# GLAD-RUC/DistEGNN

Hardware: NVIDIA H100
Metric: graph_steps_per_sec (higher is better)
Workload: dtype f32

## Files before the change

distegnn_b200/csrc/tc16.cuh:

```cuda
#pragma once
#include <cuda_fp16.h>

#include <type_traits>

#include "common.cuh"
#include "tile_mma.cuh"

namespace degnn {
namespace tc16 {

constexpr float RANGE = 3.0e4f;
__device__ __forceinline__ void split_pair(f32x2 x, uint32_t& hi, uint32_t& lo) {
    float x0, x1, l0, l1;
    upk2(x, x0, x1);
    const __half2 h = __floats2half2_rn(x0, x1);
    hi = *reinterpret_cast<const uint32_t*>(&h);
    const float2 hf = __half22float2(h);
    upk2(sub2(x, pk2(hf.x, hf.y)), l0, l1);
    const __half2 l = __floats2half2_rn(l0, l1);
    lo = *reinterpret_cast<const uint32_t*>(&l);
}

template <int NTHREADS, bool TRANSPOSED = false>
__device__ __forceinline__ void stage_weight(__half* hi, __half* lo, const float* __restrict__ wt_kmajor, int n_off,
                                             int n_total, int tid, float scale = 1.0f) {
    static_assert((H * H) % NTHREADS == 0, "thread count must divide the matrix");
    constexpr int R = H * H / NTHREADS;
    const uint32_t lbo_h = (uint32_t)(n_total / 8) * 64u;
    float w[R];
#pragma unroll
    for (int r = 0; r < R; ++r) w[r] = __ldg(wt_kmajor + tid + r * NTHREADS);
#pragma unroll
    for (int r = 0; r < R; ++r) {
        const int i = tid + r * NTHREADS;
        const int k = TRANSPOSED ? i & 63 : i >> 6, n = (TRANSPOSED ? i >> 6 : i & 63) + n_off;
        const float ws = w[r] * scale;
        const __half h = __float2half_rn(ws);
        const uint32_t o = (uint32_t)(k >> 3) * lbo_h + (uint32_t)(n >> 3) * 64u + (uint32_t)(n & 7) * 8u + (k & 7);
        hi[o] = h;
        lo[o] = __float2half_rn(ws - __half2float(h));
    }
}
__host__ __device__ constexpr uint32_t lbo_bytes(int n_total) { return (uint32_t)(n_total / 8) * 128u; }

template <uint32_t LBO, bool ACCUMULATE = false>
__device__ __forceinline__ void mma_f16x3_rA(float (&d)[32], const uint32_t (&a_hi)[16], const uint32_t (&a_lo)[16],
                                             uint64_t b_hi, uint64_t b_lo) {
    constexpr uint64_t B_KSTEP = (2 * LBO) >> 4;
    auto mma = [&](auto acc, const uint32_t (&a)[16], int ks, uint64_t b) {
        tmma::wgmma_f16_m64n64k16_rA<decltype(acc)::value>(d, a[4 * ks], a[4 * ks + 1], a[4 * ks + 2], a[4 * ks + 3],
                                                            b + ks * B_KSTEP);
    };
    tmma::wgmma_fence();
    mma(std::integral_constant<bool, ACCUMULATE>{}, a_lo, 0, b_hi);
#pragma unroll
    for (int ks = 1; ks < 4; ++ks) mma(std::true_type{}, a_lo, ks, b_hi);
#pragma unroll
    for (int ks = 0; ks < 4; ++ks) mma(std::true_type{}, a_hi, ks, b_lo);
#pragma unroll
    for (int ks = 0; ks < 4; ++ks) mma(std::true_type{}, a_hi, ks, b_hi);
    tmma::wgmma_commit();
}
__device__ __forceinline__ void mma_f16x3_rA_wait(float (&d)[32], uint32_t (&a_hi)[16], uint32_t (&a_lo)[16]) {
    tmma::wgmma_wait_all();
#pragma unroll
    for (int i = 0; i < 32; ++i) tmma::wgmma_keep(d[i]);
#pragma unroll
    for (int i = 0; i < 16; ++i) {
        tmma::wgmma_keep(a_hi[i]);
        tmma::wgmma_keep(a_lo[i]);
    }
}

__device__ __forceinline__ bool row_overflow(__half2 mx) {
    return fmaxf(__low2float(mx), __high2float(mx)) > RANGE;
}
__device__ __forceinline__ float range_scale(float rowmax) {
    const uint32_t eb = (__float_as_uint(rowmax) >> 23) & 0xffu;
    const uint32_t sb = eb > 141u ? 268u - eb : 127u;
    return __uint_as_float((sb < 1u ? 1u : sb) << 23);
}
__device__ __forceinline__ float quad_max(float v) {
    v = fmaxf(v, __shfl_xor_sync(FULL, v, 1));
    return fmaxf(v, __shfl_xor_sync(FULL, v, 2));
}
__device__ __forceinline__ float quad_sum(float v) {
    v += __shfl_xor_sync(FULL, v, 1);
    return v + __shfl_xor_sync(FULL, v, 2);
}

struct RowScales {
    float a = 1.0f, b = 1.0f, inv_a = 1.0f, inv_b = 1.0f;
};
constexpr int FAST_PASS = 0, MAX_PASS = 1, ENCODE_PASS = 2;
template <int P>
using Pass = std::integral_constant<int, P>;
struct NoGuard {
    __device__ __forceinline__ bool operator()() const { return false; }
};

template <bool SCALES_IN, bool ROLLED_MAX = false, class F, class Guard = NoGuard>
__device__ __forceinline__ void encode_rows(F&& f, uint32_t (&hi)[16], uint32_t (&lo)[16], RowScales& s,
                                            Guard&& guard = Guard{}) {
    bool cold = SCALES_IN && __any_sync(FULL, s.a != 1.0f || s.b != 1.0f);
    if (!cold) {
        __half2 mx = __floats2half2_rn(0.f, 0.f);
#pragma unroll
        for (int j = 0; j < 8; ++j) {
            f32x2 xa, xb;
            f(j, xa, xb, Pass<FAST_PASS>{});
            split_pair(xa, hi[2 * j], lo[2 * j]);
            split_pair(xb, hi[2 * j + 1], lo[2 * j + 1]);
            mx = __hmax2(mx, __habs2(*reinterpret_cast<const __half2*>(&hi[2 * j])));
            mx = __hmax2(mx, __habs2(*reinterpret_cast<const __half2*>(&hi[2 * j + 1])));
        }
        cold = __any_sync(FULL, row_overflow(mx) || guard());
    }
    if (!cold) return;
    float fa = 0.f, fb = 0.f;
    auto row_max = [&](int j) {
        f32x2 xa, xb;
        float v0, v1;
        f(j, xa, xb, Pass<MAX_PASS>{});
        upk2(xa, v0, v1);
        fa = fmaxf(fa, fmaxf(fabsf(v0), fabsf(v1)));
        upk2(xb, v0, v1);
        fb = fmaxf(fb, fmaxf(fabsf(v0), fabsf(v1)));
    };
    if constexpr (ROLLED_MAX) {
#pragma unroll 1
        for (int j = 0; j < 8; ++j) row_max(j);
    } else {
#pragma unroll
        for (int j = 0; j < 8; ++j) row_max(j);
    }
    float ca = range_scale(quad_max(fa)), ia = 1.0f / ca;
    float cb = range_scale(quad_max(fb)), ib = 1.0f / cb;
    if constexpr (SCALES_IN) {
        ca = fminf(ca, s.a);
        cb = fminf(cb, s.b);
        ia = 1.0f / ca;
        ib = 1.0f / cb;
    }
    s = {ca, cb, ia, ib};
#pragma unroll
    for (int j = 0; j < 8; ++j) {
        f32x2 xa, xb;
        f(j, xa, xb, Pass<ENCODE_PASS>{});
        split_pair(mul2(xa, bc2(s.a)), hi[2 * j], lo[2 * j]);
        split_pair(mul2(xb, bc2(s.b)), hi[2 * j + 1], lo[2 * j + 1]);
    }
}

__device__ __forceinline__ void phi_head_t(const float (&d)[32], float inv_a, float inv_b, const float* b, const float* w,
                                           int q, float& phia, float& phib) {
    float qmax = 0.f;
    f32x2 pha, phb;
    auto pass = [&](auto safe) {
        pha = phb = bc2(0.f);
#pragma unroll
        for (int j = 0; j < 8; ++j) {
            const f32x2 bb = *reinterpret_cast<const f32x2*>(b + 8 * j + 2 * q);
            const f32x2 ww = *reinterpret_cast<const f32x2*>(w + 8 * j + 2 * q);
            f32x2 sa = fma2(pk2(d[4 * j + 0], d[4 * j + 1]), bc2(inv_a), bb);
            f32x2 sb = fma2(pk2(d[4 * j + 2], d[4 * j + 3]), bc2(inv_b), bb);
            silu4t<decltype(safe)::value>(sa, sb, qmax);
            pha = fma2(sa, ww, pha);
            phb = fma2(sb, ww, phb);
        }
    };
    pass(std::false_type{});
    if (__any_sync(FULL, silu_q_overflow(qmax))) pass(std::true_type{});
    float p0, p1;
    upk2(pha, p0, p1);
    phia = quad_sum(p0 + p1);
    upk2(phb, p0, p1);
    phib = quad_sum(p0 + p1);
}

}
}
```

distegnn_b200/csrc/tile_mma.cuh:

```cuda
#pragma once
#include <cuda_runtime.h>
#include <stdint.h>

namespace degnn {

extern __shared__ __align__(1024) uint8_t degnn_dyn_smem[];

namespace tmma {

constexpr uint32_t TM_COLGROUP_BYTES = 2048;
__host__ __device__ constexpr int tm_bytes(int ncols) { return ncols * 128 * 4; }

__device__ __forceinline__ uint32_t smem_u32(const void* p) {
    return (uint32_t)__cvta_generic_to_shared(p);
}

__device__ __forceinline__ uint32_t tm_addr_rc(uint32_t row, uint32_t col) {
    return smem_u32(degnn_dyn_smem) + (col >> 2) * TM_COLGROUP_BYTES + row * 16u + (col & 3u) * 4u;
}
__device__ __forceinline__ uint32_t tm_addr(uint32_t taddr) {
    return tm_addr_rc((taddr >> 16) + (threadIdx.x & 31u), taddr & 0xffffu);
}

__device__ __forceinline__ uint64_t make_desc(uint32_t smem_addr, uint32_t lbo, uint32_t sbo) {
    return (uint64_t)((smem_addr >> 4) & 0x3FFF) | ((uint64_t)((lbo >> 4) & 0x3FFF) << 16) |
           ((uint64_t)((sbo >> 4) & 0x3FFF) << 32);
}

__device__ __forceinline__ void fence_proxy_async_smem() { asm volatile("fence.proxy.async.shared::cta;" ::: "memory"); }

__device__ __forceinline__ void tm_st4(uint32_t taddr, const uint32_t (&r)[4]) {
    asm volatile("st.shared.v4.b32 [%0], {%1,%2,%3,%4};" ::"r"(tm_addr(taddr)), "r"(r[0]), "r"(r[1]), "r"(r[2]), "r"(r[3])
                 : "memory");
}
__device__ __forceinline__ void tm_ld4(uint32_t taddr, uint32_t* r) {
    asm volatile("ld.shared.v4.b32 {%0,%1,%2,%3}, [%4];" : "=r"(r[0]), "=r"(r[1]), "=r"(r[2]), "=r"(r[3]) : "r"(tm_addr(taddr))
                 : "memory");
}
__device__ __forceinline__ void tm_st8(uint32_t taddr, const uint32_t (&r)[8]) {
    tm_st4(taddr, *reinterpret_cast<const uint32_t(*)[4]>(&r[0]));
    tm_st4(taddr + 4, *reinterpret_cast<const uint32_t(*)[4]>(&r[4]));
}
__device__ __forceinline__ void tm_st16(uint32_t taddr, const uint32_t (&r)[16]) {
#pragma unroll
    for (int i = 0; i < 4; ++i) tm_st4(taddr + 4 * i, *reinterpret_cast<const uint32_t(*)[4]>(&r[4 * i]));
}
__device__ __forceinline__ void tm_ld16(uint32_t taddr, uint32_t (&r)[16]) {
#pragma unroll
    for (int i = 0; i < 4; ++i) tm_ld4(taddr + 4 * i, &r[4 * i]);
}
__device__ __forceinline__ void prefetch_l1(const void* p) { asm volatile("prefetch.global.L1 [%0];" ::"l"(p)); }
__device__ __forceinline__ void prefetch_l2(const void* p) { asm volatile("prefetch.global.L2 [%0];" ::"l"(p)); }

__device__ __forceinline__ void wgmma_fence() { asm volatile("wgmma.fence.sync.aligned;" ::: "memory"); }
__device__ __forceinline__ void wgmma_commit() { asm volatile("wgmma.commit_group.sync.aligned;" ::: "memory"); }
__device__ __forceinline__ void wgmma_wait_all() { asm volatile("wgmma.wait_group.sync.aligned 0;" ::: "memory"); }
__device__ __forceinline__ void wgmma_f16_m64n64k16(float (&d)[32], uint64_t a_desc, uint64_t b_desc, uint32_t accumulate) {
    asm volatile(
        "{\n\t"
        ".reg .pred p;\n\t"
        "setp.ne.b32 p, %34, 0;\n\t"
        "wgmma.mma_async.sync.aligned.m64n64k16.f32.f16.f16 "
        "{%0,%1,%2,%3,%4,%5,%6,%7,%8,%9,%10,%11,%12,%13,%14,%15,%16,%17,%18,%19,%20,%21,%22,%23,%24,%25,%26,%27,%28,%29,%30,%31},"
        " %32, %33, p, 1, 1, 0, 0;\n\t"
        "}\n"
        : "+f"(d[0]), "+f"(d[1]), "+f"(d[2]), "+f"(d[3]), "+f"(d[4]), "+f"(d[5]), "+f"(d[6]), "+f"(d[7]), "+f"(d[8]),
          "+f"(d[9]), "+f"(d[10]), "+f"(d[11]), "+f"(d[12]), "+f"(d[13]), "+f"(d[14]), "+f"(d[15]), "+f"(d[16]),
          "+f"(d[17]), "+f"(d[18]), "+f"(d[19]), "+f"(d[20]), "+f"(d[21]), "+f"(d[22]), "+f"(d[23]), "+f"(d[24]),
          "+f"(d[25]), "+f"(d[26]), "+f"(d[27]), "+f"(d[28]), "+f"(d[29]), "+f"(d[30]), "+f"(d[31])
        : "l"(a_desc), "l"(b_desc), "r"(accumulate)
        : "memory");
}
#define DEGNN_WGMMA_RA_D(c)                                                                                             \
    c(d[0]), c(d[1]), c(d[2]), c(d[3]), c(d[4]), c(d[5]), c(d[6]), c(d[7]), c(d[8]), c(d[9]), c(d[10]), c(d[11]),      \
        c(d[12]), c(d[13]), c(d[14]), c(d[15]), c(d[16]), c(d[17]), c(d[18]), c(d[19]), c(d[20]), c(d[21]), c(d[22]),  \
        c(d[23]), c(d[24]), c(d[25]), c(d[26]), c(d[27]), c(d[28]), c(d[29]), c(d[30]), c(d[31])
#define DEGNN_WGMMA_RA_ASM(scale_d)                                                                                     \
    "wgmma.mma_async.sync.aligned.m64n64k16.f32.f16.f16 "                                                               \
    "{%0,%1,%2,%3,%4,%5,%6,%7,%8,%9,%10,%11,%12,%13,%14,%15,%16,%17,%18,%19,%20,%21,%22,%23,%24,%25,%26,%27,%28,%29,%30," \
    "%31}, {%32,%33,%34,%35}, %36, " scale_d ", 1, 1, 0;\n"
template <bool ACCUMULATE>
__device__ __forceinline__ void wgmma_f16_m64n64k16_rA(float (&d)[32], uint32_t a0, uint32_t a1, uint32_t a2, uint32_t a3,
                                                       uint64_t b_desc) {
    if (ACCUMULATE)
        asm volatile(DEGNN_WGMMA_RA_ASM("1") : DEGNN_WGMMA_RA_D("+f")
                     : "r"(a0), "r"(a1), "r"(a2), "r"(a3), "l"(b_desc) : "memory");
    else
        asm volatile(DEGNN_WGMMA_RA_ASM("0") : DEGNN_WGMMA_RA_D("=f")
                     : "r"(a0), "r"(a1), "r"(a2), "r"(a3), "l"(b_desc) : "memory");
}
#undef DEGNN_WGMMA_RA_D
#undef DEGNN_WGMMA_RA_ASM
__device__ __forceinline__ void wgmma_keep(float& r) { asm volatile("" : "+f"(r)::"memory"); }
__device__ __forceinline__ void wgmma_keep(uint32_t& r) { asm volatile("" : "+r"(r)::"memory"); }
__device__ __forceinline__ void frag_rows(int mb, uint32_t& r0, uint32_t& q) {
    const uint32_t w = (threadIdx.x >> 5) & 3u, l = threadIdx.x & 31u;
    r0 = 64u * (uint32_t)mb + 16u * w + (l >> 2);
    q = l & 3u;
}
__device__ __forceinline__ void frag_store(const float (&d)[32], uint32_t col, int mb) {
    uint32_t r0, q;
    frag_rows(mb, r0, q);
#pragma unroll
    for (int j = 0; j < 8; ++j) {
        const uint32_t c = col + 8u * j + 2u * q;
        const uint32_t a0 = tm_addr_rc(r0, c), a1 = tm_addr_rc(r0 + 8u, c);
        asm volatile("st.shared.v2.f32 [%0], {%1,%2};" ::"r"(a0), "f"(d[4 * j]), "f"(d[4 * j + 1]) : "memory");
        asm volatile("st.shared.v2.f32 [%0], {%1,%2};" ::"r"(a1), "f"(d[4 * j + 2]), "f"(d[4 * j + 3]) : "memory");
    }
}
__device__ __forceinline__ void frag_load(float (&d)[32], uint32_t col, int mb) {
    uint32_t r0, q;
    frag_rows(mb, r0, q);
#pragma unroll
    for (int j = 0; j < 8; ++j) {
        const uint32_t c = col + 8u * j + 2u * q;
        asm volatile("ld.shared.v2.f32 {%0,%1}, [%2];" : "=f"(d[4 * j]), "=f"(d[4 * j + 1]) : "r"(tm_addr_rc(r0, c)) : "memory");
        asm volatile("ld.shared.v2.f32 {%0,%1}, [%2];" : "=f"(d[4 * j + 2]), "=f"(d[4 * j + 3]) : "r"(tm_addr_rc(r0 + 8u, c))
                     : "memory");
    }
}

__device__ __forceinline__ void mbar_init(uint64_t* bar, uint32_t count) {
    asm volatile("mbarrier.init.shared::cta.b64 [%0], %1;" ::"r"(smem_u32(bar)), "r"(count) : "memory");
}
__device__ __forceinline__ void fence_mbar_init() { asm volatile("fence.mbarrier_init.release.cluster;" ::: "memory"); }
__device__ __forceinline__ void mbar_expect_tx(uint64_t* bar, uint32_t bytes) {
    asm volatile("mbarrier.arrive.expect_tx.shared::cta.b64 _, [%0], %1;" ::"r"(smem_u32(bar)), "r"(bytes) : "memory");
}
__device__ __forceinline__ void mbar_wait(uint64_t* bar, uint32_t parity) {
    asm volatile(
        "{\n\t"
        ".reg .pred p;\n\t"
        "WAIT_LOOP:\n\t"
        "mbarrier.try_wait.parity.shared::cta.b64 p, [%0], %1;\n\t"
        "@p bra WAIT_DONE;\n\t"
        "bra WAIT_LOOP;\n\t"
        "WAIT_DONE:\n\t"
        "}\n" ::"r"(smem_u32(bar)),
        "r"(parity)
        : "memory");
}

__device__ __forceinline__ void bulk_g2s(void* smem_dst, const void* gsrc, uint32_t bytes, uint64_t* bar) {
    asm volatile("cp.async.bulk.shared::cluster.global.mbarrier::complete_tx::bytes [%0], [%1], %2, [%3];" ::"r"(
                     smem_u32(smem_dst)),
                 "l"(gsrc), "r"(bytes), "r"(smem_u32(bar))
                 : "memory");
}

__device__ __forceinline__ void cp_async16(uint32_t smem_addr, const void* gsrc) {
    asm volatile("cp.async.cg.shared.global [%0], [%1], 16;" ::"r"(smem_addr), "l"(gsrc) : "memory");
}
__device__ __forceinline__ void cp_async16(void* smem_dst, const void* gsrc) { cp_async16(smem_u32(smem_dst), gsrc); }
__device__ __forceinline__ void cp_async8(void* smem_dst, const void* gsrc) {
    asm volatile("cp.async.ca.shared.global [%0], [%1], 8;" ::"r"(smem_u32(smem_dst)), "l"(gsrc) : "memory");
}
__device__ __forceinline__ void cp_async4(void* smem_dst, const void* gsrc) {
    asm volatile("cp.async.ca.shared.global [%0], [%1], 4;" ::"r"(smem_u32(smem_dst)), "l"(gsrc) : "memory");
}
__device__ __forceinline__ void cp_async_commit() { asm volatile("cp.async.commit_group;" ::: "memory"); }
__device__ __forceinline__ void cp_async_wait_all() { asm volatile("cp.async.wait_group 0;" ::: "memory"); }
__device__ __forceinline__ void red_add_v2(float* gdst, float a, float b) {
    asm volatile("red.global.add.v2.f32 [%0], {%1, %2};" ::"l"(gdst), "f"(a), "f"(b) : "memory");
}

__device__ __forceinline__ void named_bar(uint32_t id, uint32_t nthreads) {
    asm volatile("bar.sync %0, %1;" ::"r"(id), "r"(nthreads) : "memory");
}

}
}
```

distegnn_b200/csrc/virtual_layer_tc16.cu:

```cuda
#include "common.cuh"
#include "det.cuh"
#include "tc16.cuh"
#include "tile_mma.cuh"

namespace degnn {

struct VirtT16Args {
    int64_t N;
    int B;
    unsigned flags;
    const int32_t* batch;
    const float* x4;
    const float* Hn;
    const float* Xv;
    const float* G;
    const float* w1r;
    const float* w2; const float* b2;
    const float* wxv; const float* bxv; const float* w3xv;
    const float* wx; const float* bx; const float* w3x;
    float* agg_v;
    float* trans_v;
    float* vsum;
    float* slots;
    int chunk_shift;
};

constexpr int VW_WG = 4;
constexpr int VW_THREADS = 128 * VW_WG, VW_WARPS = VW_THREADS / 32;
constexpr int VW_TILE = 64;
constexpr int VW_ROW = 72;
constexpr int VW_W = 64 * 64;
constexpr uint32_t VW_LBO = 1024;
__host__ __device__ constexpr int vw_smem_floats(int C) {
    return 6 * VW_W / 2 + 6 * H + VW_WARPS * 16 * VW_ROW + VW_WG * VW_TILE * 6 + VW_WG * C * VW_ROW + VW_WARPS * C * H
           + VW_WARPS * 4 * C;
}
__host__ __device__ constexpr int vw_smem_bytes(int C) { return vw_smem_floats(C) * 4; }

static_assert(VW_TILE == DET_VTILE, "det.cuh sizes the slots from the tile");
template <int C, bool DET>
__global__ void __launch_bounds__(VW_THREADS, 1) virtual_layer_t16_kernel(const VirtT16Args a) {
    using namespace tmma;
    __half* W2hi = reinterpret_cast<__half*>(degnn_dyn_smem);
    __half* W2lo = W2hi + VW_W;
    __half* Wxvhi = W2lo + VW_W;
    __half* Wxvlo = Wxvhi + VW_W;
    __half* Wxhi = Wxvlo + VW_W;
    __half* Wxlo = Wxhi + VW_W;
    float* w1rs = reinterpret_cast<float*>(Wxlo + VW_W);
    float* b2s = w1rs + H;
    float* bxvs = b2s + H;
    float* w3xvs = bxvs + H;
    float* bxs = w3xvs + H;
    float* w3xs = bxs + H;
    float* stage_all = w3xs + H;
    float* dX_all = stage_all + VW_WARPS * 16 * VW_ROW;
    float* phi_all = dX_all + VW_WG * VW_TILE * 4;
    float* gs_all = phi_all + VW_WG * VW_TILE * 2;
    float* accH_all = gs_all + VW_WG * C * VW_ROW;
    float* accX_all = accH_all + VW_WARPS * C * H;

    const int tid = threadIdx.x;
    const int lane = tid & 31;
    const int warp = tid >> 5;
    const int wg = warp >> 2;
    const int w = warp & 3;
    const int t = tid & 127;
    const int g = lane >> 2, q = lane & 3;
    constexpr int K = 4 + 3 * C + H * C;
    const bool need_feat = !(a.flags & DISTEGNN_FLAG_LAST);
    constexpr int TN = VW_TILE / C;
    constexpr bool warp_local = (16 % C) == 0;

    tc16::stage_weight<VW_THREADS>(W2hi, W2lo, a.w2, 0, 64, tid, SILU_T_IN);
    tc16::stage_weight<VW_THREADS>(Wxvhi, Wxvlo, a.wxv, 0, 64, tid);
    tc16::stage_weight<VW_THREADS>(Wxhi, Wxlo, a.wx, 0, 64, tid);
    if (tid < H) {
        w1rs[tid] = a.w1r[tid];
        b2s[tid] = a.b2[tid] * SILU_T_IN;
        bxvs[tid] = a.bxv[tid] * SILU_T_IN;
        w3xvs[tid] = a.w3xv[tid] * SILU_T_OUT;
        bxs[tid] = a.bx[tid] * SILU_T_IN;
        w3xs[tid] = a.w3x[tid] * SILU_T_OUT;
    }
    for (int i = tid; i < VW_WARPS * (C * H + 4 * C); i += VW_THREADS) accH_all[i] = 0.f;
    fence_proxy_async_smem();
    __syncthreads();

    const uint64_t bW0 = make_desc(smem_u32(W2hi), VW_LBO, 128);
    auto bW = [&](int k) { return bW0 + (uint64_t)(k * (VW_W * 2 / 16)); };
    float* tile_s = stage_all + wg * VW_TILE * VW_ROW;
    float* dXs = dX_all + wg * VW_TILE * 4;
    float* phis = phi_all + wg * VW_TILE * 2;
    float* gs = gs_all + wg * C * VW_ROW;
    float* accH = accH_all + warp * C * H;
    float* accX = accX_all + warp * 4 * C;
    float* accH_g = accH_all + 4 * wg * C * H;
    float* accX_g = accX_all + 4 * wg * 4 * C;
    const uint32_t bar_id = 1 + wg;
    int cur_graph = -1;

    auto flush = [&](int gr) {
        if (gr < 0) return;
        float* dst = a.vsum + (size_t)gr * K;
        if (need_feat)
            for (int i = t; i < C * H; i += 128) {
                float s = 0.f;
#pragma unroll
                for (int k = 0; k < 4; ++k) {
                    s += accH_g[k * C * H + i];
                    accH_g[k * C * H + i] = 0.f;
                }
                atomicAdd(dst + 4 + 3 * C + i, s * SILU_T_OUT);
            }
        if (t < 3 * C) {
            float s = 0.f;
#pragma unroll
            for (int k = 0; k < 4; ++k) {
                s += accX_g[k * 4 * C + t];
                accX_g[k * 4 * C + t] = 0.f;
            }
            atomicAdd(dst + 4 + t, s);
        }
    };

    const int num_tiles = (int)((a.N + TN - 1) / TN);
    const int stride = (int)gridDim.x * VW_WG;
    const int CH = 1 << a.chunk_shift;
    auto next_tile = [&](int tl) {
        if constexpr (DET) return ((tl + 1) & (CH - 1)) != 0 ? tl + 1 : tl + 1 + (stride - 1) * CH;
        else return tl + stride;
    };
    float* accG = accH_all + 4 * wg * C * H;
    float* accXG = accX_all + 4 * wg * 4 * C;
    int curM = -1, curX = -1, cont = -1;
    auto det_dst = [&](int gr, int tl) {
        return gr == cont ? a.slots + (size_t)(tl >> a.chunk_shift) * K : a.vsum + (size_t)gr * K;
    };
    auto det_flush_m = [&](int tl) {
        for (int c = t >> 5; c < C; c += 4) {
            f32x2* acc = reinterpret_cast<f32x2*>(accG + c * H + 2 * (t & 31));
            if (curM >= 0) {
                float* dst = det_dst(curM, tl) + 4 + 3 * C + c * H + 2 * (t & 31);
                upk2(mul2(*acc, bc2(SILU_T_OUT)), dst[0], dst[1]);
            }
            *acc = 0ull;
        }
    };
    auto det_flush_x = [&](int tl) {
        if (t < 3 * C) {
            if (curX >= 0) det_dst(curX, tl)[4 + t] = accXG[t];
            accXG[t] = 0.f;
        }
    };
    const int ra = 16 * w + g, rb = ra + 8;
    const float* colp = tile_s + 2 * lane;

    for (int tile = DET ? ((int)blockIdx.x * VW_WG + wg) * CH : (int)blockIdx.x * VW_WG + wg; tile < num_tiles;
         tile = next_tile(tile)) {
        const int64_t n0 = (int64_t)tile * TN;
        if (DET && (tile & (CH - 1)) == 0)
            cont = (n0 > 0 && __ldg(a.batch + n0 - 1) == __ldg(a.batch + n0)) ? __ldg(a.batch + n0) : -1;
        const int nvalid = (int)min((int64_t)TN, a.N - n0);
        const int rows = nvalid * C;
        {
            const int64_t nn0 = (int64_t)next_tile(tile) * TN;
            const int nnv = (int)min((int64_t)TN, a.N - nn0);
            for (int i = t; i < 2 * nnv; i += 128) prefetch_l1(a.Hn + (size_t)nn0 * H + 32 * i);
            if (nnv > 0) {
                if (t < (nnv * 16 + 127) / 128) prefetch_l1(a.x4 + (size_t)nn0 * 4 + 32 * t);
                if (t == 127) prefetch_l1(a.batch + nn0);
                if (t == 126) prefetch_l1(a.batch + nn0 + nnv - 1);
            }
        }
        const int g_first = __ldg(a.batch + n0), g_last = __ldg(a.batch + n0 + nvalid - 1);
        const bool single = (g_first == g_last);
        if (single && g_first != cur_graph) {
            named_bar(bar_id, 128);
            if constexpr (!DET) flush(cur_graph);
            cur_graph = g_first;
            for (int i = t; i < C * (H / 4); i += 128) {
                const int c = i / (H / 4), q4 = i - c * (H / 4);
                *reinterpret_cast<float4*>(gs + c * VW_ROW + 4 * q4) = ldg4(a.G + ((size_t)g_first * C + c) * H + 4 * q4);
            }
            named_bar(bar_id, 128);
        }

        const bool va = ra < rows, vb = rb < rows;
        const float* pa;
        const float* pb;
        const float* ga;
        const float* gb;
        float vra, vrb;
        {
            const int nla = va ? ra / C : 0, nlb = vb ? rb / C : 0;
            const int cha = va ? ra - nla * C : 0;
            const int chb = 8 % C == 0 ? cha : (vb ? rb - nlb * C : 0);
            const size_t nda = (size_t)(n0 + nla), ndb = C == 16 ? nda : (size_t)(n0 + nlb);
            const int gra = single ? g_first : __ldg(a.batch + nda);
            const int grb = (C == 16 || single) ? gra : __ldg(a.batch + ndb);
            const float4 xia = ldg4(a.x4 + nda * 4);
            const float4 xib = C == 16 ? xia : ldg4(a.x4 + ndb * 4);
            auto xv = [&](int gr, int ch) {
                const float* Xg = a.Xv + (size_t)gr * 3 * C + ch;
                return make_float3(__ldg(Xg), __ldg(Xg + C), __ldg(Xg + 2 * C));
            };
            const float3 xva = xv(gra, cha);
            const float3 xvb = (8 % C == 0 && grb == gra) ? xva : xv(grb, chb);
            auto row_geo = [&](int r, size_t node, int gr, int ch, float4 xi, float3 xg, const float*& hrow,
                               const float*& grow) {
                const float dx = xg.x - xi.x, dy = xg.y - xi.y, dz = xg.z - xi.z;
                if (q == 0) *reinterpret_cast<float4*>(dXs + 4 * r) = make_float4(dx, dy, dz, 0.f);
                hrow = a.Hn + node * H + 2 * q;
                grow = (gr == cur_graph ? (const float*)(gs + ch * VW_ROW) : a.G + ((size_t)gr * C + ch) * H) + 2 * q;
                return sqrtf(dx * dx + dy * dy + dz * dz);
            };
            vra = row_geo(ra, nda, gra, cha, xia, xva, pa, ga);
            vrb = row_geo(rb, ndb, grb, chb, xib, xvb, pb, gb);
        }
        auto pre = [&](int j, const float* hrow, const float* grow, float vr) {
            const f32x2 hh = __ldg(reinterpret_cast<const f32x2*>(hrow + 8 * j));
            const f32x2 gg = *reinterpret_cast<const f32x2*>(grow + 8 * j);
            return fma2(bc2(vr), *reinterpret_cast<const f32x2*>(w1rs + 8 * j + 2 * q), add2(hh, gg));
        };
        uint32_t ahi[16], alo[16];
        float qmax = 0.f;
        auto silu_guard = [&] { return silu_q_overflow(qmax); };
        tc16::RowScales s1;
        tc16::encode_rows<false, true>(
            [&](int j, f32x2& xa, f32x2& xb, auto pass) {
                xa = pre(j, pa, ga, vra);
                xb = pre(j, pb, gb, vrb);
                silu4p<decltype(pass)::value != tc16::FAST_PASS>(xa, xb, qmax);
                if (!va) xa = 0ull;
                if (!vb) xb = 0ull;
            },
            ahi, alo, s1, silu_guard);

        float d[32];
        tc16::mma_f16x3_rA<VW_LBO>(d, ahi, alo, bW(0), bW(1));
        tc16::mma_f16x3_rA_wait(d, ahi, alo);

        qmax = 0.f;
        tc16::RowScales s2;
        tc16::encode_rows<false>(
            [&](int j, f32x2& ma, f32x2& mb, auto pass) {
                const f32x2 bb = *reinterpret_cast<const f32x2*>(b2s + 8 * j + 2 * q);
                ma = fma2(pk2(d[4 * j + 0], d[4 * j + 1]), bc2(s1.inv_a), bb);
                mb = fma2(pk2(d[4 * j + 2], d[4 * j + 3]), bc2(s1.inv_b), bb);
                silu4t<decltype(pass)::value != tc16::FAST_PASS>(ma, mb, qmax);
                if (decltype(pass)::value != tc16::ENCODE_PASS) {
                    *reinterpret_cast<f32x2*>(tile_s + ra * VW_ROW + 8 * j + 2 * q) = ma;
                    *reinterpret_cast<f32x2*>(tile_s + rb * VW_ROW + 8 * j + 2 * q) = mb;
                }
            },
            ahi, alo, s2, silu_guard);

        const int nb = warp_local ? (16 * w) / C : w;
        const int ne = warp_local ? min(nb + 16 / C, nvalid) : nvalid;
        const int ns = warp_local ? 1 : 4;
        const int r_end = min(16 * w + 16, rows);

        tc16::mma_f16x3_rA<VW_LBO>(d, ahi, alo, bW(2), bW(3));
        if (need_feat) {
            if (warp_local && !DET) __syncwarp();
            else named_bar(bar_id, 128);
            auto ld2 = [](const float* p) { return *reinterpret_cast<const f32x2*>(p); };
            const f32x2 invC2 = bc2(SILU_T_OUT / (float)C);
#pragma unroll 1
            for (int n = nb; n < ne; n += ns) {
                const float* base = colp + (n * C) * VW_ROW;
                f32x2 s0 = 0ull, s1 = 0ull;
#pragma unroll
                for (int c = 0; c + 1 < C; c += 2) {
                    s0 = add2(s0, ld2(base + c * VW_ROW));
                    s1 = add2(s1, ld2(base + (c + 1) * VW_ROW));
                }
                if constexpr (C % 2 == 1) s0 = add2(s0, ld2(base + (C - 1) * VW_ROW));
                *reinterpret_cast<f32x2*>(a.agg_v + (size_t)(n0 + n) * H + 2 * lane) = mul2(add2(s0, s1), invC2);
            }
            if constexpr (DET) {
                for (int n = 0; n < nvalid; ++n) {
                    const int gr = single ? g_first : __ldg(a.batch + n0 + n);
                    if (gr != curM) {
                        det_flush_m(tile);
                        curM = gr;
                    }
#pragma unroll
                    for (int c = t >> 5; c < C; c += 4) {
                        f32x2* acc = reinterpret_cast<f32x2*>(accG + c * H + 2 * (t & 31));
                        *acc = add2(*acc, ld2(tile_s + (n * C + c) * VW_ROW + 2 * (t & 31)));
                    }
                }
            } else if (single) {
#pragma unroll 1
                for (int i = 0; i < C; ++i) {
                    const int r = 16 * w + i;
                    if (r >= r_end) break;
                    f32x2 s = ld2(colp + r * VW_ROW);
#pragma unroll
                    for (int k = 1; k < (16 - i + C - 1) / C; ++k)
                        if (r + k * C < r_end) s = add2(s, ld2(colp + (r + k * C) * VW_ROW));
                    f32x2* acc = reinterpret_cast<f32x2*>(accH + (r % C) * H + 2 * lane);
                    *acc = add2(*acc, s);
                }
            } else {
#pragma unroll 1
                for (int r = 16 * w; r < r_end; ++r) {
                    const int n = r / C, c = r - n * C;
                    float* dst = a.vsum + (size_t)__ldg(a.batch + n0 + n) * K + 4 + 3 * C + c * H + 2 * lane;
                    float v0, v1;
                    upk2(ld2(colp + r * VW_ROW), v0, v1);
                    atomicAdd(dst, v0 * SILU_T_OUT);
                    atomicAdd(dst + 1, v1 * SILU_T_OUT);
                }
            }
        }
        tc16::mma_f16x3_rA_wait(d, ahi, alo);

        {
            float phia, phib;
            tc16::phi_head_t(d, s2.inv_a, s2.inv_b, bxvs, w3xvs, q, phia, phib);
            if (q == 0) {
                phis[ra] = phia;
                phis[rb] = phib;
            }
        }

#pragma unroll
        for (int j = 0; j < 8; ++j) {
            const f32x2 ma = *reinterpret_cast<const f32x2*>(tile_s + ra * VW_ROW + 8 * j + 2 * q);
            const f32x2 mb = *reinterpret_cast<const f32x2*>(tile_s + rb * VW_ROW + 8 * j + 2 * q);
            tc16::split_pair(mul2(ma, bc2(s2.a)), ahi[2 * j], alo[2 * j]);
            tc16::split_pair(mul2(mb, bc2(s2.b)), ahi[2 * j + 1], alo[2 * j + 1]);
        }
        tc16::mma_f16x3_rA<VW_LBO>(d, ahi, alo, bW(4), bW(5));
        if (warp_local) __syncwarp();
        else named_bar(bar_id, 128);
        for (int i = lane; i < (ne - nb + ns - 1) / ns * 3; i += 32) {
            const int n = nb + (i / 3) * ns, dd = i - 3 * (i / 3);
            float s = 0.f;
#pragma unroll 8
            for (int c = 0; c < C; ++c) s = fmaf(-dXs[4 * (n * C + c) + dd], phis[n * C + c], s);
            a.trans_v[(size_t)(n0 + n) * 4 + dd] = s / (float)C;
        }
        tc16::mma_f16x3_rA_wait(d, ahi, alo);

        {
            float phia, phib;
            tc16::phi_head_t(d, s2.inv_a, s2.inv_b, bxs, w3xs, q, phia, phib);
            if (q == 0) {
                phis[VW_TILE + ra] = phia;
                phis[VW_TILE + rb] = phib;
            }
        }
        __syncwarp();
        const float* phx = phis + VW_TILE;
        if constexpr (DET) {
            named_bar(bar_id, 128);
            if (t < 3 * C) {
                const int dd = t / C, c = t - dd * C;
                for (int n = 0; n < nvalid; ++n) {
                    const int gr = single ? g_first : __ldg(a.batch + n0 + n);
                    if (gr != curX) {
                        det_flush_x(tile);
                        curX = gr;
                    }
                    accXG[t] = fmaf(dXs[4 * (n * C + c) + dd], phx[n * C + c], accXG[t]);
                }
            }
        } else if (single) {
            for (int it = lane; it < 3 * C; it += 32) {
                const int dd = it / C, i = it - dd * C, r = 16 * w + i;
                if (r < r_end) {
                    float s = 0.f;
#pragma unroll
                    for (int k = 0; k < (16 + C - 1) / C; ++k)
                        if (r + k * C < r_end) s = fmaf(dXs[4 * (r + k * C) + dd], phx[r + k * C], s);
                    accX[dd * C + r % C] += s;
                }
            }
        } else {
            for (int it = lane; it < 48; it += 32) {
                const int r = 16 * w + it / 3, dd = it - 3 * (it / 3);
                if (r < r_end) {
                    const int n = r / C, c = r - n * C;
                    atomicAdd(a.vsum + (size_t)__ldg(a.batch + n0 + n) * K + 4 + dd * C + c, dXs[4 * r + dd] * phx[r]);
                }
            }
        }
        if (warp_local && !DET) __syncwarp();
        else named_bar(bar_id, 128);
        if (DET && (((tile + 1) & (CH - 1)) == 0 || tile + 1 >= num_tiles)) {
            if (need_feat) det_flush_m(tile);
            det_flush_x(tile);
            curM = curX = -1;
        }
    }
    if constexpr (!DET) {
        named_bar(bar_id, 128);
        flush(cur_graph);
    }
}

}

namespace degnn {

template <bool DET, int C = 1>
static void launch_virtual(int c, unsigned grid, const VirtT16Args& a, cudaStream_t stream) {
    if constexpr (C <= DISTEGNN_MAX_CHANNELS) {
        if (c != C) return launch_virtual<DET, C + 1>(c, grid, a, stream);
        static_assert(vw_smem_bytes(C) <= 232448, "the shared memory of every C must fit");
        ensure_dynamic_smem((const void*)virtual_layer_t16_kernel<C, DET>, vw_smem_bytes(C));
        virtual_layer_t16_kernel<C, DET><<<grid, VW_THREADS, vw_smem_bytes(C), stream>>>(a);
    }
}

template <bool DET>
static int virtual_layer_fwd(int64_t n_nodes, int n_graphs, int A, int C, int Na, unsigned flags, const int32_t* batch32,
                             const float* x4, const float* Hn, const float* Xv, const float* G, const float* layer_params,
                             float* agg_v, float* trans_v, float* vsum, void* workspace, int64_t workspace_bytes,
                             void* stream, int max_ctas) {
    if (int rc = check_dims(A, C, Na)) return rc;
    if (n_nodes == 0) return DISTEGNN_OK;
    DEGNN_CHECK_ARG(n_nodes > 0 && n_graphs > 0, "bad size");
    DEGNN_CHECK_ARG(batch32 && x4 && Hn && Xv && G && layer_params && trans_v && vsum, "null pointer");
    DEGNN_CHECK_ARG((flags & DISTEGNN_FLAG_LAST) || agg_v, "null agg_v");
    if (DET)
        if (int rc = det_check_workspace(n_nodes, -1, C, workspace, workspace_bytes, "distegnn_virtual_layer_fwd_det"))
            return rc;
    Layout L = make_layout(A, C, Na);
    VirtT16Args a;
    a.N = n_nodes; a.B = n_graphs; a.flags = flags;
    a.batch = batch32; a.x4 = x4; a.Hn = Hn; a.Xv = Xv; a.G = G;
    a.w1r = layer_params + L.off[DISTEGNN_P_V_W1R];
    a.w2 = layer_params + L.off[DISTEGNN_P_V_W2];
    a.b2 = layer_params + L.off[DISTEGNN_P_V_B2];
    a.wxv = layer_params + L.off[DISTEGNN_P_V_WXV];
    a.bxv = layer_params + L.off[DISTEGNN_P_V_BXV];
    a.w3xv = layer_params + L.off[DISTEGNN_P_V_W3XV];
    a.wx = layer_params + L.off[DISTEGNN_P_V_WX];
    a.bx = layer_params + L.off[DISTEGNN_P_V_BX];
    a.w3x = layer_params + L.off[DISTEGNN_P_V_W3X];
    a.agg_v = agg_v; a.trans_v = trans_v; a.vsum = vsum;
    a.slots = DET ? det_vsum_slots(workspace) : nullptr;
    a.chunk_shift = DET ? det_chunk_shift(n_nodes, C) : 0;
    const int TN = VW_TILE / C;
    const int64_t tiles = (n_nodes + TN - 1) / TN;
    const int64_t units = DET ? det_chunks(n_nodes, C) : tiles;
    DEGNN_CHECK_ARG(tiles + ((int64_t)sm_count() * VW_WG << (DET ? det_chunk_shift(n_nodes, C) : 0)) < ((int64_t)1 << 31),
                    "too many nodes");
    int64_t grid = (units + VW_WG - 1) / VW_WG;
    if (grid > sm_count()) grid = sm_count();
    if (DET) grid = det_grid(grid, max_ctas);
    launch_virtual<DET>(C, (unsigned)grid, a, (cudaStream_t)stream);
    DEGNN_CHECK_LAUNCH();
    return DISTEGNN_OK;
}

int virtual_layer_fwd_det(int64_t n_nodes, int n_graphs, int A, int C, int Na, unsigned flags, const int32_t* batch32,
                          const float* x4, const float* Hn, const float* Xv, const float* G, const float* layer_params,
                          float* agg_v, float* trans_v, float* vsum, void* workspace, int64_t workspace_bytes,
                          void* stream, int max_ctas) {
    return virtual_layer_fwd<true>(n_nodes, n_graphs, A, C, Na, flags, batch32, x4, Hn, Xv, G, layer_params, agg_v,
                                   trans_v, vsum, workspace, workspace_bytes, stream, max_ctas);
}

}

extern "C" int distegnn_virtual_layer_fwd(int64_t n_nodes, int n_graphs, int A, int C, int Na, unsigned flags,
                                          const int32_t* batch32, const float* x4, const float* Hn,
                                          const float* Xv, const float* G, const float* layer_params,
                                          float* agg_v, float* trans_v, float* vsum, void* stream) {
    return degnn::virtual_layer_fwd<false>(n_nodes, n_graphs, A, C, Na, flags, batch32, x4, Hn, Xv, G, layer_params,
                                           agg_v, trans_v, vsum, nullptr, 0, stream, 0);
}

extern "C" int distegnn_virtual_layer_fwd_det(int64_t n_nodes, int n_graphs, int A, int C, int Na, unsigned flags,
                                              const int32_t* batch32, const float* x4, const float* Hn,
                                              const float* Xv, const float* G, const float* layer_params,
                                              float* agg_v, float* trans_v, float* vsum, void* workspace,
                                              int64_t workspace_bytes, void* stream) {
    return degnn::virtual_layer_fwd_det(n_nodes, n_graphs, A, C, Na, flags, batch32, x4, Hn, Xv, G, layer_params,
                                        agg_v, trans_v, vsum, workspace, workspace_bytes, stream, 0);
}
```

Measured before the change: 37.84.

## Stage message tile as swizzled fp16 hi/lo image and pool via wgmma

Replaces the fp32 message staging tile with a swizzled fp16 hi/lo shared-memory image written straight from the encoded A fragments. The next projection reads its A operand from shared memory through descriptors instead of re-splitting, and, when unscaled and the tile is full, the per-node mean pooling runs as a wgmma against a 0/1 selection matrix. This removes the fp32 staging traffic and the repeated split work, in exchange for more shared memory, a block-wide OR barrier, and fp16 pooling that is only exact up to the hi/lo split.

```diff
diff --git a/distegnn_b200/csrc/tc16.cuh b/distegnn_b200/csrc/tc16.cuh
--- a/distegnn_b200/csrc/tc16.cuh
+++ b/distegnn_b200/csrc/tc16.cuh
@@ -70,6 +70,24 @@
         tmma::wgmma_keep(a_hi[i]);
         tmma::wgmma_keep(a_lo[i]);
     }
+}
+
+template <uint32_t LBO>
+__device__ __forceinline__ void mma_f16x3_sA(float (&d)[32], uint64_t a_hi, uint64_t a_lo, uint64_t b_hi, uint64_t b_lo) {
+    constexpr uint64_t B_KSTEP = (2 * LBO) >> 4, A_KSTEP = 32 >> 4;
+    tmma::wgmma_fence();
+#pragma unroll
+    for (int ks = 0; ks < 4; ++ks) tmma::wgmma_f16_m64n64k16(d, a_lo + ks * A_KSTEP, b_hi + ks * B_KSTEP, ks > 0);
+#pragma unroll
+    for (int ks = 0; ks < 4; ++ks) tmma::wgmma_f16_m64n64k16(d, a_hi + ks * A_KSTEP, b_lo + ks * B_KSTEP, 1);
+#pragma unroll
+    for (int ks = 0; ks < 4; ++ks) tmma::wgmma_f16_m64n64k16(d, a_hi + ks * A_KSTEP, b_hi + ks * B_KSTEP, 1);
+    tmma::wgmma_commit();
+}
+__device__ __forceinline__ void mma_f16x3_sA_wait(float (&d)[32]) {
+    tmma::wgmma_wait_all();
+#pragma unroll
+    for (int i = 0; i < 32; ++i) tmma::wgmma_keep(d[i]);
 }
 
 __device__ __forceinline__ bool row_overflow(__half2 mx) {
diff --git a/distegnn_b200/csrc/tile_mma.cuh b/distegnn_b200/csrc/tile_mma.cuh
--- a/distegnn_b200/csrc/tile_mma.cuh
+++ b/distegnn_b200/csrc/tile_mma.cuh
@@ -91,6 +91,51 @@
 }
 #undef DEGNN_WGMMA_RA_D
 #undef DEGNN_WGMMA_RA_ASM
+#define DEGNN_WGMMA_TA_ASM(n, regs, a, b, scale_d) \
+    "wgmma.mma_async.sync.aligned.m64n" n "k16.f32.f16.f16 {" regs "}, " a ", " b ", " scale_d ", 1, 1, 1, 0;\n"
+#define DEGNN_R8 "%0,%1,%2,%3,%4,%5,%6,%7"
+#define DEGNN_R12 DEGNN_R8 ",%8,%9,%10,%11"
+#define DEGNN_R20 DEGNN_R12 ",%12,%13,%14,%15,%16,%17,%18,%19"
+#define DEGNN_D8(c) c(d[0]), c(d[1]), c(d[2]), c(d[3]), c(d[4]), c(d[5]), c(d[6]), c(d[7])
+#define DEGNN_D12(c) DEGNN_D8(c), c(d[8]), c(d[9]), c(d[10]), c(d[11])
+#define DEGNN_D20(c) DEGNN_D12(c), c(d[12]), c(d[13]), c(d[14]), c(d[15]), c(d[16]), c(d[17]), c(d[18]), c(d[19])
+template <int N, bool ACCUMULATE>
+__device__ __forceinline__ void wgmma_f16_m64nNk16_tA(float (&d)[N / 2], uint64_t a_desc, uint64_t b_desc) {
+    static_assert(N == 16 || N == 24 || N == 40, "instantiated for N = 16, 24, 40");
+    if constexpr (N == 16) {
+        if constexpr (ACCUMULATE)
+            asm volatile(DEGNN_WGMMA_TA_ASM("16", DEGNN_R8, "%8", "%9", "1") : DEGNN_D8("+f") : "l"(a_desc), "l"(b_desc)
+                         : "memory");
+        else
+            asm volatile(DEGNN_WGMMA_TA_ASM("16", DEGNN_R8, "%8", "%9", "0") : DEGNN_D8("=f") : "l"(a_desc), "l"(b_desc)
+                         : "memory");
+    } else if constexpr (N == 24) {
+        if constexpr (ACCUMULATE)
+            asm volatile(DEGNN_WGMMA_TA_ASM("24", DEGNN_R12, "%12", "%13", "1") : DEGNN_D12("+f")
+                         : "l"(a_desc), "l"(b_desc) : "memory");
+        else
+            asm volatile(DEGNN_WGMMA_TA_ASM("24", DEGNN_R12, "%12", "%13", "0") : DEGNN_D12("=f")
+                         : "l"(a_desc), "l"(b_desc) : "memory");
+    } else {
+        if constexpr (ACCUMULATE)
+            asm volatile(DEGNN_WGMMA_TA_ASM("40", DEGNN_R20, "%20", "%21", "1") : DEGNN_D20("+f")
+                         : "l"(a_desc), "l"(b_desc) : "memory");
+        else
+            asm volatile(DEGNN_WGMMA_TA_ASM("40", DEGNN_R20, "%20", "%21", "0") : DEGNN_D20("=f")
+                         : "l"(a_desc), "l"(b_desc) : "memory");
+    }
+}
+#undef DEGNN_WGMMA_TA_ASM
+#undef DEGNN_R8
+#undef DEGNN_R12
+#undef DEGNN_R20
+#undef DEGNN_D8
+#undef DEGNN_D12
+#undef DEGNN_D20
+__device__ __forceinline__ uint64_t make_desc_sw128(uint32_t smem_addr) {
+    return make_desc(smem_addr, 16, 1024) | (1ull << 62);
+}
+
 __device__ __forceinline__ void wgmma_keep(float& r) { asm volatile("" : "+f"(r)::"memory"); }
 __device__ __forceinline__ void wgmma_keep(uint32_t& r) { asm volatile("" : "+r"(r)::"memory"); }
 __device__ __forceinline__ void frag_rows(int mb, uint32_t& r0, uint32_t& q) {
@@ -168,6 +213,20 @@
 __device__ __forceinline__ void named_bar(uint32_t id, uint32_t nthreads) {
     asm volatile("bar.sync %0, %1;" ::"r"(id), "r"(nthreads) : "memory");
 }
-
-}
-}
+__device__ __forceinline__ bool named_bar_any(uint32_t id, uint32_t nthreads, bool pred) {
+    uint32_t r;
+    asm volatile(
+        "{\n\t"
+        ".reg .pred p, q;\n\t"
+        "setp.ne.u32 p, %1, 0;\n\t"
+        "bar.red.or.pred q, %2, %3, p;\n\t"
+        "selp.u32 %0, 1, 0, q;\n\t"
+        "}\n"
+        : "=r"(r)
+        : "r"((uint32_t)pred), "r"(id), "r"(nthreads)
+        : "memory");
+    return r != 0;
+}
+
+}
+}
diff --git a/distegnn_b200/csrc/virtual_layer_tc16.cu b/distegnn_b200/csrc/virtual_layer_tc16.cu
--- a/distegnn_b200/csrc/virtual_layer_tc16.cu
+++ b/distegnn_b200/csrc/virtual_layer_tc16.cu
@@ -2,6 +2,8 @@
 #include "det.cuh"
 #include "tc16.cuh"
 #include "tile_mma.cuh"
+
+#include <utility>
 
 namespace degnn {
 
@@ -31,11 +33,46 @@
 constexpr int VW_ROW = 72;
 constexpr int VW_W = 64 * 64;
 constexpr uint32_t VW_LBO = 1024;
+constexpr int VW_IMG = 64 * 32;
+__host__ __device__ constexpr int vw_pool_n(int C) { return 64 / C + C <= 64 ? (64 / C + C + 7) / 8 * 8 : 0; }
 __host__ __device__ constexpr int vw_smem_floats(int C) {
-    return 6 * VW_W / 2 + 6 * H + VW_WARPS * 16 * VW_ROW + VW_WG * VW_TILE * 6 + VW_WG * C * VW_ROW + VW_WARPS * C * H
-           + VW_WARPS * 4 * C;
+    return 6 * VW_W / 2 + VW_WG * 2 * VW_IMG + vw_pool_n(C) * 32 + 6 * H + VW_WG * VW_TILE * 6 + VW_WG * C * VW_ROW
+           + VW_WARPS * C * H + VW_WARPS * 4 * C;
 }
 __host__ __device__ constexpr int vw_smem_bytes(int C) { return vw_smem_floats(C) * 4; }
+
+template <int J>
+__device__ __forceinline__ void st_words(uint32_t wa, uint32_t ha, uint32_t la, uint32_t hb, uint32_t lb) {
+    asm volatile(
+        "{\n\t.reg .b32 p;\n\t"
+        "xor.b32 p, %0, %1;\n\t"
+        "st.shared.b32 [p], %2;\n\t"
+        "st.shared.b32 [p+%6], %3;\n\t"
+        "st.shared.b32 [p+1024], %4;\n\t"
+        "st.shared.b32 [p+%7], %5;\n\t}\n" ::"r"(wa), "n"(16 * J), "r"(ha), "r"(la), "r"(hb), "r"(lb), "n"(4 * VW_IMG),
+        "n"(4 * VW_IMG + 1024)
+        : "memory");
+}
+template <int J>
+__device__ __forceinline__ void ld_words(uint32_t wa, uint32_t& ha, uint32_t& la, uint32_t& hb, uint32_t& lb) {
+    asm volatile(
+        "{\n\t.reg .b32 p;\n\t"
+        "xor.b32 p, %4, %5;\n\t"
+        "ld.shared.b32 %0, [p];\n\t"
+        "ld.shared.b32 %1, [p+%6];\n\t"
+        "ld.shared.b32 %2, [p+1024];\n\t"
+        "ld.shared.b32 %3, [p+%7];\n\t}\n"
+        : "=r"(ha), "=r"(la), "=r"(hb), "=r"(lb)
+        : "r"(wa), "n"(16 * J), "n"(4 * VW_IMG), "n"(4 * VW_IMG + 1024)
+        : "memory");
+}
+
+template <class F, int... J>
+__device__ __forceinline__ void blocks8(F&& f, std::integer_sequence<int, J...>) {
+    (f(std::integral_constant<int, J>{}), ...);
+}
+template <class F>
+__device__ __forceinline__ void blocks8(F&& f) { blocks8(f, std::make_integer_sequence<int, 8>{}); }
 
 static_assert(VW_TILE == DET_VTILE, "det.cuh sizes the slots from the tile");
 template <int C, bool DET>
@@ -47,14 +84,15 @@
     __half* Wxvlo = Wxvhi + VW_W;
     __half* Wxhi = Wxvlo + VW_W;
     __half* Wxlo = Wxhi + VW_W;
-    float* w1rs = reinterpret_cast<float*>(Wxlo + VW_W);
+    uint32_t* img_all = reinterpret_cast<uint32_t*>(Wxlo + VW_W);
+    __half* Ss = reinterpret_cast<__half*>(img_all + VW_WG * 2 * VW_IMG);
+    float* w1rs = reinterpret_cast<float*>(Ss + vw_pool_n(C) * 64);
     float* b2s = w1rs + H;
     float* bxvs = b2s + H;
     float* w3xvs = bxvs + H;
     float* bxs = w3xvs + H;
     float* w3xs = bxs + H;
-    float* stage_all = w3xs + H;
-    float* dX_all = stage_all + VW_WARPS * 16 * VW_ROW;
+    float* dX_all = w3xs + H;
     float* phi_all = dX_all + VW_WG * VW_TILE * 4;
     float* gs_all = phi_all + VW_WG * VW_TILE * 2;
     float* accH_all = gs_all + VW_WG * C * VW_ROW;
@@ -71,10 +109,18 @@
     const bool need_feat = !(a.flags & DISTEGNN_FLAG_LAST);
     constexpr int TN = VW_TILE / C;
     constexpr bool warp_local = (16 % C) == 0;
+    constexpr int NP = vw_pool_n(C);
+    constexpr bool POOL_TC = !DET && NP > 0;
 
     tc16::stage_weight<VW_THREADS>(W2hi, W2lo, a.w2, 0, 64, tid, SILU_T_IN);
     tc16::stage_weight<VW_THREADS>(Wxvhi, Wxvlo, a.wxv, 0, 64, tid);
     tc16::stage_weight<VW_THREADS>(Wxhi, Wxlo, a.wx, 0, 64, tid);
+    if constexpr (POOL_TC)
+        for (int i = tid; i < NP * 64; i += VW_THREADS) {
+            const int o = i >> 6, k = i & 63;
+            const bool one = o < TN ? k / C == o : (o < TN + C && k < TN * C && k % C == o - TN);
+            Ss[(k >> 3) * (NP * 8) + (o >> 3) * 64 + (o & 7) * 8 + (k & 7)] = __float2half_rn(one ? 1.f : 0.f);
+        }
     if (tid < H) {
         w1rs[tid] = a.w1r[tid];
         b2s[tid] = a.b2[tid] * SILU_T_IN;
@@ -89,7 +135,7 @@
 
     const uint64_t bW0 = make_desc(smem_u32(W2hi), VW_LBO, 128);
     auto bW = [&](int k) { return bW0 + (uint64_t)(k * (VW_W * 2 / 16)); };
-    float* tile_s = stage_all + wg * VW_TILE * VW_ROW;
+    uint32_t* img = img_all + wg * 2 * VW_IMG;
     float* dXs = dX_all + wg * VW_TILE * 4;
     float* phis = phi_all + wg * VW_TILE * 2;
     float* gs = gs_all + wg * C * VW_ROW;
@@ -154,7 +200,13 @@
         }
     };
     const int ra = 16 * w + g, rb = ra + 8;
-    const float* colp = tile_s + 2 * lane;
+    const uint32_t wa = smem_u32(img + ra * 32 + q) + (g << 4);
+    auto ld2 = [&](int r) {
+        const int o = r * 32 + (((lane >> 2) ^ (r & 7)) << 2) + (lane & 3);
+        const float2 h = __half22float2(*reinterpret_cast<const __half2*>(img + o));
+        const float2 l = __half22float2(*reinterpret_cast<const __half2*>(img + VW_IMG + o));
+        return mul2(add2(pk2(h.x, h.y), pk2(l.x, l.y)), bc2(dXs[4 * r + 3]));
+    };
 
     for (int tile = DET ? ((int)blockIdx.x * VW_WG + wg) * CH : (int)blockIdx.x * VW_WG + wg; tile < num_tiles;
          tile = next_tile(tile)) {
@@ -249,10 +301,6 @@
                 ma = fma2(pk2(d[4 * j + 0], d[4 * j + 1]), bc2(s1.inv_a), bb);
                 mb = fma2(pk2(d[4 * j + 2], d[4 * j + 3]), bc2(s1.inv_b), bb);
                 silu4t<decltype(pass)::value != tc16::FAST_PASS>(ma, mb, qmax);
-                if (decltype(pass)::value != tc16::ENCODE_PASS) {
-                    *reinterpret_cast<f32x2*>(tile_s + ra * VW_ROW + 8 * j + 2 * q) = ma;
-                    *reinterpret_cast<f32x2*>(tile_s + rb * VW_ROW + 8 * j + 2 * q) = mb;
-                }
             },
             ahi, alo, s2, silu_guard);
 
@@ -262,21 +310,67 @@
         const int r_end = min(16 * w + 16, rows);
 
         tc16::mma_f16x3_rA<VW_LBO>(d, ahi, alo, bW(2), bW(3));
-        if (need_feat) {
-            if (warp_local && !DET) __syncwarp();
-            else named_bar(bar_id, 128);
-            auto ld2 = [](const float* p) { return *reinterpret_cast<const f32x2*>(p); };
+        blocks8([&](auto j) { st_words<j>(wa, ahi[2 * j], alo[2 * j], ahi[2 * j + 1], alo[2 * j + 1]); });
+        if (q == 0) {
+            dXs[4 * ra + 3] = s2.inv_a;
+            dXs[4 * rb + 3] = s2.inv_b;
+        }
+        float pd[POOL_TC ? NP / 2 : 1];
+        auto pool_issue = [&] {
+            if constexpr (POOL_TC) {
+                const uint64_t a_hi = make_desc_sw128(smem_u32(img)), a_lo = make_desc_sw128(smem_u32(img + VW_IMG));
+                const uint64_t bS = make_desc(smem_u32(Ss), NP * 16, 128);
+                wgmma_fence();
+                wgmma_f16_m64nNk16_tA<NP, false>(pd, a_lo, bS);
+#pragma unroll
+                for (int ks = 1; ks < 4; ++ks) wgmma_f16_m64nNk16_tA<NP, true>(pd, a_lo + ks * 128, bS + ks * 2 * NP);
+#pragma unroll
+                for (int ks = 0; ks < 4; ++ks) wgmma_f16_m64nNk16_tA<NP, true>(pd, a_hi + ks * 128, bS + ks * 2 * NP);
+                wgmma_commit();
+            }
+        };
+        auto pool_readout = [&] {
+            if constexpr (POOL_TC) {
+#pragma unroll
+                for (int i = 0; i < NP / 2; ++i) wgmma_keep(pd[i]);
+                const int fa = 16 * w + g;
+                const float invC = SILU_T_OUT / (float)C;
+#pragma unroll
+                for (int j = 0; j < NP / 8; ++j)
+#pragma unroll
+                    for (int e = 0; e < 2; ++e) {
+                        const int o = 8 * j + 2 * q + e;
+                        if (o < TN) {
+                            float* dst = a.agg_v + (size_t)(n0 + o) * H + fa;
+                            dst[0] = pd[4 * j + e] * invC;
+                            dst[8] = pd[4 * j + 2 + e] * invC;
+                        } else if (o < TN + C) {
+                            float* acc = accH + (o - TN) * H + fa;
+                            acc[0] += pd[4 * j + e];
+                            acc[8] += pd[4 * j + 2 + e];
+                        }
+                    }
+            }
+        };
+        fence_proxy_async_smem();
+        bool pool_tc = false;
+        if constexpr (POOL_TC) {
+            const bool scaled = named_bar_any(bar_id, 128, s2.a != 1.0f || s2.b != 1.0f);
+            pool_tc = need_feat && !scaled && single && nvalid == TN;
+        } else {
+            named_bar(bar_id, 128);
+        }
+        if (need_feat && !pool_tc) {
             const f32x2 invC2 = bc2(SILU_T_OUT / (float)C);
 #pragma unroll 1
             for (int n = nb; n < ne; n += ns) {
-                const float* base = colp + (n * C) * VW_ROW;
                 f32x2 s0 = 0ull, s1 = 0ull;
 #pragma unroll
                 for (int c = 0; c + 1 < C; c += 2) {
-                    s0 = add2(s0, ld2(base + c * VW_ROW));
-                    s1 = add2(s1, ld2(base + (c + 1) * VW_ROW));
-                }
-                if constexpr (C % 2 == 1) s0 = add2(s0, ld2(base + (C - 1) * VW_ROW));
+                    s0 = add2(s0, ld2(n * C + c));
+                    s1 = add2(s1, ld2(n * C + c + 1));
+                }
+                if constexpr (C % 2 == 1) s0 = add2(s0, ld2(n * C + C - 1));
                 *reinterpret_cast<f32x2*>(a.agg_v + (size_t)(n0 + n) * H + 2 * lane) = mul2(add2(s0, s1), invC2);
             }
             if constexpr (DET) {
@@ -286,10 +380,10 @@
                         det_flush_m(tile);
                         curM = gr;
                     }
-#pragma unroll
+#pragma unroll(C <= 8 ? 2 : 1)
                     for (int c = t >> 5; c < C; c += 4) {
                         f32x2* acc = reinterpret_cast<f32x2*>(accG + c * H + 2 * (t & 31));
-                        *acc = add2(*acc, ld2(tile_s + (n * C + c) * VW_ROW + 2 * (t & 31)));
+                        *acc = add2(*acc, ld2(n * C + c));
                     }
                 }
             } else if (single) {
@@ -297,10 +391,10 @@
                 for (int i = 0; i < C; ++i) {
                     const int r = 16 * w + i;
                     if (r >= r_end) break;
-                    f32x2 s = ld2(colp + r * VW_ROW);
+                    f32x2 s = ld2(r);
 #pragma unroll
                     for (int k = 1; k < (16 - i + C - 1) / C; ++k)
-                        if (r + k * C < r_end) s = add2(s, ld2(colp + (r + k * C) * VW_ROW));
+                        if (r + k * C < r_end) s = add2(s, ld2(r + k * C));
                     f32x2* acc = reinterpret_cast<f32x2*>(accH + (r % C) * H + 2 * lane);
                     *acc = add2(*acc, s);
                 }
@@ -310,13 +404,18 @@
                     const int n = r / C, c = r - n * C;
                     float* dst = a.vsum + (size_t)__ldg(a.batch + n0 + n) * K + 4 + 3 * C + c * H + 2 * lane;
                     float v0, v1;
-                    upk2(ld2(colp + r * VW_ROW), v0, v1);
+                    upk2(ld2(r), v0, v1);
                     atomicAdd(dst, v0 * SILU_T_OUT);
                     atomicAdd(dst + 1, v1 * SILU_T_OUT);
                 }
             }
         }
         tc16::mma_f16x3_rA_wait(d, ahi, alo);
+        if (pool_tc) {
+            pool_issue();
+            wgmma_wait_all();
+            pool_readout();
+        }
 
         {
             float phia, phib;
@@ -327,14 +426,13 @@
             }
         }
 
-#pragma unroll
-        for (int j = 0; j < 8; ++j) {
-            const f32x2 ma = *reinterpret_cast<const f32x2*>(tile_s + ra * VW_ROW + 8 * j + 2 * q);
-            const f32x2 mb = *reinterpret_cast<const f32x2*>(tile_s + rb * VW_ROW + 8 * j + 2 * q);
-            tc16::split_pair(mul2(ma, bc2(s2.a)), ahi[2 * j], alo[2 * j]);
-            tc16::split_pair(mul2(mb, bc2(s2.b)), ahi[2 * j + 1], alo[2 * j + 1]);
-        }
-        tc16::mma_f16x3_rA<VW_LBO>(d, ahi, alo, bW(4), bW(5));
+        if constexpr (DET) {
+            blocks8([&](auto j) { ld_words<j>(wa, ahi[2 * j], alo[2 * j], ahi[2 * j + 1], alo[2 * j + 1]); });
+            tc16::mma_f16x3_rA<VW_LBO>(d, ahi, alo, bW(4), bW(5));
+        } else {
+            tc16::mma_f16x3_sA<VW_LBO>(d, make_desc_sw128(smem_u32(img)), make_desc_sw128(smem_u32(img + VW_IMG)), bW(4),
+                                       bW(5));
+        }
         if (warp_local) __syncwarp();
         else named_bar(bar_id, 128);
         for (int i = lane; i < (ne - nb + ns - 1) / ns * 3; i += 32) {
@@ -344,7 +442,8 @@
             for (int c = 0; c < C; ++c) s = fmaf(-dXs[4 * (n * C + c) + dd], phis[n * C + c], s);
             a.trans_v[(size_t)(n0 + n) * 4 + dd] = s / (float)C;
         }
-        tc16::mma_f16x3_rA_wait(d, ahi, alo);
+        if constexpr (DET) tc16::mma_f16x3_rA_wait(d, ahi, alo);
+        else tc16::mma_f16x3_sA_wait(d);
 
         {
             float phia, phib;
```

Measured after the change: 38.28 (median of 6 runs). 1.01x the previous value.
